# IDEA-CCNL/Fengshenbang-LM

Measured on NVIDIA H100. Metric: tokens_per_sec, higher is better.
Workload: dtype bf16

## Files before the change

### fengshen-lm_b200/csrc/gemm.cu

```cuda
#include "host_common.h"
#include "ptx.cuh"

namespace fsb {

constexpr int GEMM_BM = 128;
constexpr int GEMM_BK = 64;
constexpr int GEMM_THREADS = 384;

struct GemmParams {
  void* D;
  void* aux;
  const void* bias;
  int64_t ldd, ldaux, stride_d, stride_aux;
  int M, N, K, batch;
  int d_f32;
  int bias_f32;
  int epilogue;
  int accumulate;
  int tiles_m, tiles_n;
  int group_m;
  int ksplits;
};

template <int BN>
struct GemmSmem {
  static constexpr int STAGES = BN == 256 ? 4 : 6;
  static constexpr int A_BYTES = GEMM_BM * GEMM_BK * 2;
  static constexpr int B_BYTES = BN * GEMM_BK * 2;
  static constexpr int STAGE_BYTES = A_BYTES + B_BYTES;
  static constexpr int EPI_BUF_BYTES = 64 * 128;
  static constexpr int EPI_OFFSET = STAGES * STAGE_BYTES;
  static constexpr int BAR_OFFSET = EPI_OFFSET + 2  * 2  * EPI_BUF_BYTES;
  static constexpr int TOTAL = BAR_OFFSET + 2 * STAGES * 8 + 1024 ;
  static_assert(TOTAL <= kSmemOptIn, "exceeds the 227 KB of shared memory a block can opt into on sm_90");
};

__device__ __forceinline__ float gelu_tanh_f(float x) {
  const float k1 = 0.044715f, c = -2.f * 0.7978845608028654f * 1.4426950408889634f;
  const float t = ex2_approx(c * x * fmaf(k1, x * x, 1.f));
  return __fdividef(x, 1.f + t);
}
__device__ __forceinline__ float gelu_erf_f(float x) {
  const float z = fabsf(x) * 0.7071067811865476f;
  const float t = __fdividef(1.f, fmaf(0.3275911f, z, 1.f));
  float pl = fmaf(t, 1.061405429f, -1.453152027f);
  pl = fmaf(t, pl, 1.421413741f);
  pl = fmaf(t, pl, -0.284496736f);
  pl = fmaf(t, pl, 0.254829592f);
  const float erfc_z = pl * t * ex2_approx(-1.4426950408889634f * z * z);
  const float hx = 0.5f * x;
  return x >= 0.f ? fmaf(-hx, erfc_z, x) : hx * erfc_z;
}

__device__ __forceinline__ void tile_coords(int t, int tiles_m, int tiles_n, int group_m, int& b, int& m_idx, int& n_idx) {
  const int per = tiles_m * tiles_n;
  b = t / per;
  int r = t - b * per;
  const int group_span = group_m * tiles_n;
  const int g = r / group_span;
  const int first_m = g * group_m;
  const int gsize = min(tiles_m - first_m, group_m);
  const int in_g = r - g * group_span;
  m_idx = first_m + in_g % gsize;
  n_idx = in_g / gsize;
}

__device__ __forceinline__ void k_range(const GemmParams& p, int b, int num_kb, int& kb_lo, int& kb_hi, int& ab) {
  if (p.ksplits > 1) {
    kb_lo = int(int64_t(b) * num_kb / p.ksplits);
    kb_hi = int(int64_t(b + 1) * num_kb / p.ksplits);
    ab = 0;
  } else {
    kb_lo = 0; kb_hi = num_kb; ab = b;
  }
}

template <int kLayout, int BN>
__global__ void __launch_bounds__(GEMM_THREADS, 1)
gemm_bf16_kernel(const __grid_constant__ CUtensorMap tmA, const __grid_constant__ CUtensorMap tmB,
                 const __grid_constant__ CUtensorMap tmD, const __grid_constant__ CUtensorMap tmAux, const GemmParams p) {
  constexpr bool A_MN = (kLayout == FSB_GEMM_TN);
  constexpr bool B_MN = (kLayout != FSB_GEMM_NT);
  using S = GemmSmem<BN>;

  extern __shared__ uint8_t smem_raw[];
  uint8_t* smem = align_smem_1024(smem_raw);
  TmaRing<S::STAGES> ring(reinterpret_cast<uint64_t*>(smem + S::BAR_OFFSET));

  const int warp = threadIdx.x >> 5;
  const int lane = threadIdx.x & 31;
  const int num_tiles = p.tiles_m * p.tiles_n * p.batch;
  const int num_kb = (p.K + GEMM_BK - 1) / GEMM_BK;

  if (threadIdx.x == 0) {
    tma_prefetch_desc(&tmA);
    tma_prefetch_desc(&tmB);
    ring.init();
    fence_barrier_init();
  }
  if (threadIdx.x == 128) {
    tma_prefetch_desc(&tmD);
    if (p.aux != nullptr) tma_prefetch_desc(&tmAux);
  }
  __syncthreads();

  if (warp < 4) {
    reg_dec<40>();
    if (threadIdx.x == 0) {
      for (int t = blockIdx.x; t < num_tiles; t += gridDim.x) {
        int b, m_idx, n_idx, kb_lo, kb_hi, ab;
        tile_coords(t, p.tiles_m, p.tiles_n, p.group_m, b, m_idx, n_idx);
        k_range(p, b, num_kb, kb_lo, kb_hi, ab);
        const int m0 = m_idx * GEMM_BM, n0 = n_idx * BN;
        for (int kb = kb_lo; kb < kb_hi; ++kb) {
          ring.acquire();
          uint8_t* sa = smem + ring.stage * S::STAGE_BYTES;
          uint8_t* sb = sa + S::A_BYTES;
          uint64_t* bar = ring.expect(S::STAGE_BYTES);
          const int k0 = kb * GEMM_BK;
          if constexpr (!A_MN) {
            tma_load_3d(sa, &tmA, bar, k0, m0, ab);
          } else {
#pragma unroll
            for (int c = 0; c < GEMM_BM / 64; ++c)
              tma_load_3d(sa + c * (GEMM_BK * 128), &tmA, bar, m0 + c * 64, k0, ab);
          }
          if constexpr (!B_MN) {
            tma_load_3d(sb, &tmB, bar, k0, n0, ab);
          } else {
#pragma unroll
            for (int c = 0; c < BN / 64; ++c)
              tma_load_3d(sb + c * (GEMM_BK * 128), &tmB, bar, n0 + c * 64, k0, ab);
          }
          ring.advance();
        }
      }
    }
  } else {
    reg_inc<232>();
    const int wg = (threadIdx.x >> 7) - 1;
    const int wl = warp & 3;
    const bool leader = (threadIdx.x & 127) == 0;
    const uint64_t dsc_a = A_MN ? make_smem_desc_sw128(smem_u32(smem) + wg * (GEMM_BK * 128), GEMM_BK * 128, 1024)
                                : make_smem_desc_sw128(smem_u32(smem) + wg * (64 * 128), 0, 1024);
    const uint64_t dsc_b = B_MN ? make_smem_desc_sw128(smem_u32(smem) + S::A_BYTES, GEMM_BK * 128, 1024)
                                : make_smem_desc_sw128(smem_u32(smem) + S::A_BYTES, 0, 1024);
    uint8_t* const epi_buf = smem + S::EPI_OFFSET + wg * (2 * S::EPI_BUF_BYTES);
    uint32_t n_stored = 0;
    float acc[BN / 2];
    for (int t = blockIdx.x; t < num_tiles; t += gridDim.x) {
      int b, m_idx, n_idx, kb_lo, kb_hi, ab;
      tile_coords(t, p.tiles_m, p.tiles_n, p.group_m, b, m_idx, n_idx);
      k_range(p, b, num_kb, kb_lo, kb_hi, ab);
      int prev = 0;
      for (int kb = kb_lo; kb < kb_hi; ++kb) {
        ring.wait();
        const uint64_t so = uint64_t(ring.stage) * (S::STAGE_BYTES >> 4);
        wgmma_fence();
#pragma unroll
        for (int k = 0; k < GEMM_BK / 16; ++k) {
          const uint64_t da = dsc_a + so + ((A_MN ? k * 2048 : k * 32) >> 4), db = dsc_b + so + ((B_MN ? k * 2048 : k * 32) >> 4);
          const uint32_t accum = (kb != kb_lo || k != 0) ? 1u : 0u;
          if constexpr (BN == 256) wgmma_ss_n256<A_MN, B_MN>(acc, da, db, accum);
          else wgmma_ss_n128<A_MN, B_MN>(acc, da, db, accum);
        }
        wgmma_commit();
        wgmma_wait<1>();
        if (kb > kb_lo) ring.release(prev, lane);
        prev = ring.stage;
        ring.advance();
      }
      wgmma_wait<0>();
      wgmma_fence_acc(acc);
      ring.release(prev, lane);

      const int r = wl * 16 + (lane >> 2);
      const int m0 = m_idx * GEMM_BM + wg * 64, n0 = n_idx * BN;
      const int64_t d_off = int64_t(b) * p.stride_d;
      auto stage_out = [&](const CUtensorMap* tm, int c0, auto&& fill) {
        uint8_t* buf = epi_buf + (n_stored & 1) * S::EPI_BUF_BYTES;
        if (leader) tma_store_wait_read<1>();
        bar_sync(1 + wg, 128);
        fill(buf);
        fence_proxy_async();
        bar_sync(1 + wg, 128);
        if (leader) {
          tma_store_3d(tm, buf, c0, m0, b);
          tma_store_commit();
        }
        ++n_stored;
      };
#pragma unroll
      for (int j = 0; j < BN / 8; ++j) {
        const int col = n0 + 8 * j + 2 * (lane & 3);
        float bv0 = 0.f, bv1 = 0.f;
        if (p.bias != nullptr) {
          if (p.bias_f32) {
            if (col < p.N) bv0 = __ldg(reinterpret_cast<const float*>(p.bias) + col);
            if (col + 1 < p.N) bv1 = __ldg(reinterpret_cast<const float*>(p.bias) + col + 1);
          } else {
            if (col < p.N) bv0 = __bfloat162float(__ldg(reinterpret_cast<const __nv_bfloat16*>(p.bias) + col));
            if (col + 1 < p.N) bv1 = __bfloat162float(__ldg(reinterpret_cast<const __nv_bfloat16*>(p.bias) + col + 1));
          }
        }
        acc[4 * j] += bv0; acc[4 * j + 1] += bv1; acc[4 * j + 2] += bv0; acc[4 * j + 3] += bv1;
      }
#pragma unroll
      for (int g = 0; g < BN / 64; ++g) {
        if (p.aux != nullptr) {
          stage_out(&tmAux, n0 + 64 * g, [&](uint8_t* buf) {
#pragma unroll
            for (int jj = 0; jj < 8; ++jj)
#pragma unroll
              for (int h = 0; h < 2; ++h) {
                const int j = 8 * g + jj;
                *reinterpret_cast<uint32_t*>(buf + swz128(r + 8 * h, 16 * jj + 4 * (lane & 3))) =
                    pack_bf16x2(acc[4 * j + 2 * h], acc[4 * j + 2 * h + 1]);
              }
          });
        }
#pragma unroll
        for (int i = 32 * g; i < 32 * g + 32; ++i) {
          if (p.epilogue == FSB_EPI_GELU_TANH) acc[i] = gelu_tanh_f(acc[i]);
          else if (p.epilogue == FSB_EPI_GELU_ERF) acc[i] = gelu_erf_f(acc[i]);
        }
        if (p.accumulate) {
#pragma unroll
          for (int jj = 0; jj < 8; ++jj) {
            const int j = 8 * g + jj;
            const int col = n0 + 8 * j + 2 * (lane & 3);
#pragma unroll
            for (int h = 0; h < 2; ++h) {
              const int row = m0 + r + 8 * h;
              if (row >= p.M || col >= p.N) continue;
              const bool two = col + 1 < p.N;
              const int64_t o = d_off + int64_t(row) * p.ldd + col;
              if (p.d_f32) {
                const float* dp = reinterpret_cast<const float*>(p.D) + o;
                if (two) { const float2 q = *reinterpret_cast<const float2*>(dp); acc[4 * j + 2 * h] += q.x; acc[4 * j + 2 * h + 1] += q.y; }
                else acc[4 * j + 2 * h] += *dp;
              } else {
                const __nv_bfloat16* dp = reinterpret_cast<const __nv_bfloat16*>(p.D) + o;
                if (two) { const uint32_t q = *reinterpret_cast<const uint32_t*>(dp); acc[4 * j + 2 * h] += bf16lo(q); acc[4 * j + 2 * h + 1] += bf16hi(q); }
                else acc[4 * j + 2 * h] += __bfloat162float(*dp);
              }
            }
          }
        }
        if (p.d_f32) {
#pragma unroll
          for (int q = 0; q < 2; ++q)
            stage_out(&tmD, n0 + 64 * g + 32 * q, [&](uint8_t* buf) {
#pragma unroll
              for (int jj = 0; jj < 4; ++jj)
#pragma unroll
                for (int h = 0; h < 2; ++h) {
                  const int j = 8 * g + 4 * q + jj;
                  *reinterpret_cast<float2*>(buf + swz128(r + 8 * h, 32 * jj + 8 * (lane & 3))) =
                      make_float2(acc[4 * j + 2 * h], acc[4 * j + 2 * h + 1]);
                }
            });
        } else {
          stage_out(&tmD, n0 + 64 * g, [&](uint8_t* buf) {
#pragma unroll
            for (int jj = 0; jj < 8; ++jj)
#pragma unroll
              for (int h = 0; h < 2; ++h) {
                const int j = 8 * g + jj;
                *reinterpret_cast<uint32_t*>(buf + swz128(r + 8 * h, 16 * jj + 4 * (lane & 3))) =
                    pack_bf16x2(acc[4 * j + 2 * h], acc[4 * j + 2 * h + 1]);
              }
          });
        }
      }
    }
    if (leader) tma_store_wait<0>();
  }
}

static int g_reserved_sms = 0;
static inline int gemm_sms() {
  const int n = num_sms() - g_reserved_sms;
  return n < 1 ? 1 : n;
}

template <int kLayout, int BN>
static int launch_gemm(const CUtensorMap& tmA, const CUtensorMap& tmB, const CUtensorMap& tmD, const CUtensorMap& tmAux,
                       const GemmParams& p, cudaStream_t stream) {
  using S = GemmSmem<BN>;
  if (int rc = ensure_smem<gemm_bf16_kernel<kLayout, BN>>(S::TOTAL, "gemm")) return rc;
  const int num_tiles = p.tiles_m * p.tiles_n * p.batch;
  const int grid = num_tiles < gemm_sms() ? num_tiles : gemm_sms();
  gemm_bf16_kernel<kLayout, BN><<<grid, GEMM_THREADS, S::TOTAL, stream>>>(tmA, tmB, tmD, tmAux, p);
  FSB_CUDA_LAUNCH_CHECK();
  return FSB_OK;
}

struct GemmPlan {
  int bn, splits;
};
static GemmPlan gemm_plan(int layout, int64_t M, int64_t N, int64_t K, int64_t batch, bool plain, int sms) {
  const int64_t tiles256 = ((M + GEMM_BM - 1) / GEMM_BM) * ((N + 255) / 256) * batch;
  const int bn = (N > 128 && tiles256 * 10 >= int64_t(sms) * 7) ? 256 : 128;
  if (!(layout == FSB_GEMM_TN && batch == 1 && plain && N % 4 == 0 && (M * N) % 8 == 0 && K >= 4096)) return {bn, 1};
  const bool wide = N >= 256;
  const int64_t tiles = ((M + GEMM_BM - 1) / GEMM_BM) * (wide ? (N + 255) / 256 : (N + 127) / 128);
  int splits = int(sms / tiles);
  if (splits > 16) splits = 16;
  while (splits > 1 && (K % (int64_t(splits) * GEMM_BK) != 0 || K / splits < 1024)) --splits;
  if (splits >= 2 && tiles * 2 <= sms) return {wide ? 256 : bn, splits};
  return {bn, 1};
}

__global__ void splitk_reduce_kernel(const float* __restrict__ ws, int splits, int64_t M, int64_t N, void* D, int64_t ldd,
                                     int d_f32, int accumulate) {
  const int64_t n4 = N / 4;
  for (int64_t i = blockIdx.x * int64_t(blockDim.x) + threadIdx.x; i < M * n4; i += int64_t(gridDim.x) * blockDim.x) {
    const int64_t m = i / n4, n = (i - m * n4) * 4;
    float4 acc = *reinterpret_cast<const float4*>(ws + m * N + n);
    for (int s = 1; s < splits; ++s) {
      const float4 v = *reinterpret_cast<const float4*>(ws + (int64_t(s) * M + m) * N + n);
      acc.x += v.x; acc.y += v.y; acc.z += v.z; acc.w += v.w;
    }
    if (d_f32) {
      float4* dp = reinterpret_cast<float4*>(reinterpret_cast<float*>(D) + m * ldd + n);
      if (accumulate) { const float4 o = *dp; acc.x += o.x; acc.y += o.y; acc.z += o.z; acc.w += o.w; }
      *dp = acc;
    } else {
      uint2* dp = reinterpret_cast<uint2*>(reinterpret_cast<__nv_bfloat16*>(D) + m * ldd + n);
      if (accumulate) {
        const uint2 o = *dp;
        acc.x += bf16lo(o.x); acc.y += bf16hi(o.x); acc.z += bf16lo(o.y); acc.w += bf16hi(o.y);
      }
      *dp = make_uint2(pack_bf16x2(acc.x, acc.y), pack_bf16x2(acc.z, acc.w));
    }
  }
}

static int gemm_impl(int layout, int64_t M, int64_t N, int64_t K, const void* A, int64_t lda, const void* B,
                     int64_t ldb, void* D, int64_t ldd, int d_dtype, const void* bias, int bias_dtype,
                     int epilogue, int accumulate, void* aux, int64_t ldaux, int64_t batch, int64_t stride_a,
                     int64_t stride_b, int64_t stride_d, int64_t stride_aux, cudaStream_t stream, int bn = 0,
                     int ksplits = 1);

}

using namespace fsb;

extern "C" int fsb_set_reserved_sms(int n) {
  FSB_REQUIRE(n >= 0 && n <= 64, "set_reserved_sms: %d out of range [0, 64]", n);
  fsb::g_reserved_sms = n;
  return FSB_OK;
}

extern "C" size_t fsb_gemm_workspace_bytes(int layout, int64_t M, int64_t N, int64_t K) {
  if (M <= 0 || N <= 0 || K <= 0) return 0;
  const int splits = gemm_plan(layout, M, N, K, 1, true, gemm_sms()).splits;
  return splits > 1 ? size_t(splits) * size_t(M) * size_t(N) * sizeof(float) : 0;
}

extern "C" int fsb_gemm_bf16(int layout, int64_t M, int64_t N, int64_t K, const void* A, int64_t lda, const void* B,
                             int64_t ldb, void* D, int64_t ldd, int d_dtype, const void* bias, int bias_dtype,
                             int epilogue, int accumulate, void* aux, int64_t ldaux, int64_t batch, int64_t stride_a,
                             int64_t stride_b, int64_t stride_d, int64_t stride_aux, void* workspace,
                             size_t workspace_bytes, fsb_stream_t stream_) {
  cudaStream_t stream = static_cast<cudaStream_t>(stream_);
  FSB_REQUIRE(M > 0 && N > 0 && K > 0 && batch > 0, "gemm: non-positive dims M=%ld N=%ld K=%ld batch=%ld", (long)M,
              (long)N, (long)K, (long)batch);
  const GemmPlan plan = gemm_plan(layout, M, N, K, batch, bias == nullptr && aux == nullptr && epilogue == FSB_EPI_NONE,
                                  gemm_sms());
  if (plan.splits > 1 && (d_dtype == FSB_BF16 || d_dtype == FSB_F32)) {
    const int splits = plan.splits;
    const size_t need = size_t(splits) * size_t(M) * size_t(N) * sizeof(float);
    FSB_REQUIRE(workspace != nullptr && workspace_bytes >= need && aligned16(workspace),
                "gemm: this TN call splits K %d ways and needs a %zu-byte workspace (fsb_gemm_workspace_bytes); got %zu",
                splits, need, workspace_bytes);
    FSB_REQUIRE(ldd % 4 == 0, "gemm: ldd=%ld not vector-aligned", (long)ldd);
    float* ws = static_cast<float*>(workspace);
    int rc = gemm_impl(layout, M, N, K, A, lda, B, ldb, ws, N, FSB_F32, nullptr, FSB_BF16, FSB_EPI_NONE, 0, nullptr, 0,
                       splits, 0, 0, M * N, 0, stream, plan.bn, splits);
    if (rc) return rc;
    const int64_t work = M * (N / 4);
    const int blocks = int(work / 256 + 1 < 2 * num_sms() ? work / 256 + 1 : 2 * num_sms());
    splitk_reduce_kernel<<<blocks, 256, 0, stream>>>(ws, splits, M, N, D, ldd, d_dtype == FSB_F32, accumulate);
    FSB_CUDA_LAUNCH_CHECK();
    return FSB_OK;
  }
  return gemm_impl(layout, M, N, K, A, lda, B, ldb, D, ldd, d_dtype, bias, bias_dtype, epilogue, accumulate, aux, ldaux, batch,
                   stride_a, stride_b, stride_d, stride_aux, stream, plan.bn, 1);
}

static int fsb::gemm_impl(int layout, int64_t M, int64_t N, int64_t K, const void* A, int64_t lda, const void* B,
                          int64_t ldb, void* D, int64_t ldd, int d_dtype, const void* bias, int bias_dtype,
                          int epilogue, int accumulate, void* aux, int64_t ldaux, int64_t batch, int64_t stride_a,
                          int64_t stride_b, int64_t stride_d, int64_t stride_aux, cudaStream_t stream, int bn,
                          int ksplits) {
  FSB_REQUIRE(layout >= 0 && layout <= 2, "gemm: bad layout %d", layout);
  FSB_REQUIRE(M > 0 && N > 0 && K > 0 && batch > 0, "gemm: non-positive dims M=%ld N=%ld K=%ld batch=%ld", (long)M,
              (long)N, (long)K, (long)batch);
  FSB_REQUIRE(M < (1 << 30) && N < (1 << 30) && K < (1 << 30), "gemm: dims too large");
  FSB_REQUIRE(A && B && D, "gemm: null operand");
  FSB_REQUIRE(aligned16(A) && aligned16(B) && aligned16(D), "gemm: operands must be 16-byte aligned");
  FSB_REQUIRE(lda % 8 == 0 && ldb % 8 == 0, "gemm: lda/ldb must be multiples of 8 (lda=%ld ldb=%ld)", (long)lda,
              (long)ldb);
  FSB_REQUIRE(d_dtype == FSB_BF16 || d_dtype == FSB_F32, "gemm: bad d_dtype");
  FSB_REQUIRE(ldd % (d_dtype == FSB_F32 ? 4 : 8) == 0, "gemm: ldd=%ld not vector-aligned", (long)ldd);
  FSB_REQUIRE(epilogue >= 0 && epilogue <= 2, "gemm: bad epilogue %d", epilogue);
  FSB_REQUIRE(aux == nullptr || (aligned16(aux) && ldaux % 8 == 0), "gemm: aux misaligned");
  FSB_REQUIRE(batch == 1 || (stride_a % 8 == 0 && stride_b % 8 == 0 && stride_d % 8 == 0),
              "gemm: batch strides must be multiples of 8");
  FSB_REQUIRE(aux == nullptr || batch == 1 || stride_aux % 8 == 0, "gemm: aux batch stride must be a multiple of 8");
  FSB_REQUIRE(ksplits == 1 || (ksplits > 1 && ksplits <= (K + GEMM_BK - 1) / GEMM_BK && ksplits == batch),
              "gemm: bad K-split count %d", ksplits);

  CUtensorMap tmA, tmB, tmD, tmAux;
  const bool a_mn = (layout == FSB_GEMM_TN), b_mn = (layout != FSB_GEMM_NT);
  const int BN = bn ? bn : gemm_plan(layout, M, N, K, batch, false, gemm_sms()).bn;
  const int64_t ab = ksplits > 1 ? 1 : batch;
  {
    uint64_t dims[3] = {uint64_t(a_mn ? M : K), uint64_t(a_mn ? K : M), uint64_t(ab)};
    uint64_t strides[2] = {uint64_t(lda) * 2, uint64_t(ab > 1 ? stride_a : (a_mn ? K : M) * lda) * 2};
    uint32_t box[3] = {64, uint32_t(a_mn ? GEMM_BK : GEMM_BM), 1};
    int rc = make_tmap_bf16(&tmA, A, 3, dims, strides, box);
    if (rc) return rc;
  }
  {
    uint64_t dims[3] = {uint64_t(b_mn ? N : K), uint64_t(b_mn ? K : N), uint64_t(ab)};
    uint64_t strides[2] = {uint64_t(ldb) * 2, uint64_t(ab > 1 ? stride_b : (b_mn ? K : N) * ldb) * 2};
    uint32_t box[3] = {64, uint32_t(b_mn ? GEMM_BK : BN), 1};
    int rc = make_tmap_bf16(&tmB, B, 3, dims, strides, box);
    if (rc) return rc;
  }
  {
    const int64_t es = d_dtype == FSB_F32 ? 4 : 2;
    uint64_t dims[3] = {uint64_t(N), uint64_t(M), uint64_t(batch)};
    uint64_t strides[2] = {uint64_t(ldd * es), uint64_t((batch > 1 ? stride_d : M * ldd) * es)};
    uint32_t box[3] = {uint32_t(128 / es), 64, 1};
    int rc = d_dtype == FSB_F32 ? make_tmap_f32(&tmD, D, 3, dims, strides, box) : make_tmap_bf16(&tmD, D, 3, dims, strides, box);
    if (rc) return rc;
    if (aux != nullptr) {
      uint64_t astrides[2] = {uint64_t(ldaux * 2), uint64_t((batch > 1 ? stride_aux : M * ldaux) * 2)};
      uint32_t abox[3] = {64, 64, 1};
      rc = make_tmap_bf16(&tmAux, aux, 3, dims, astrides, abox);
      if (rc) return rc;
    } else {
      tmAux = tmD;
    }
  }
  GemmParams p;
  p.D = D; p.aux = aux; p.bias = bias;
  p.ldd = ldd; p.ldaux = ldaux; p.stride_d = stride_d; p.stride_aux = stride_aux;
  p.M = int(M); p.N = int(N); p.K = int(K); p.batch = int(batch);
  p.d_f32 = (d_dtype == FSB_F32); p.bias_f32 = (bias_dtype == FSB_F32);
  p.epilogue = epilogue; p.accumulate = accumulate;
  p.ksplits = ksplits;
  p.tiles_m = int((M + GEMM_BM - 1) / GEMM_BM);
  p.tiles_n = int((N + BN - 1) / BN);
  {
    const int64_t a_panel = int64_t(GEMM_BM) * (K / ksplits) * 2;
    const int64_t base = BN == 256 ? 16 : 12;
    int64_t gm = (int64_t(32) << 20) / a_panel;
    gm = gm < base ? base : (gm > 64 ? 64 : gm);
    p.group_m = int(gm);
  }

#define FSB_GEMM_DISPATCH(L) \
  case L:                    \
    return BN == 256 ? launch_gemm<L, 256>(tmA, tmB, tmD, tmAux, p, stream) : launch_gemm<L, 128>(tmA, tmB, tmD, tmAux, p, stream);
  switch (layout) {
    FSB_GEMM_DISPATCH(FSB_GEMM_NT)
    FSB_GEMM_DISPATCH(FSB_GEMM_NN)
    FSB_GEMM_DISPATCH(FSB_GEMM_TN)
  }
#undef FSB_GEMM_DISPATCH
  return FSB_ERR_INVALID;
}
```

### fengshen-lm_b200/csrc/ptx.cuh

```cuda
#pragma once
#include <cuda.h>
#include <cuda_bf16.h>
#include <cuda_runtime.h>
#include <stdint.h>

namespace fsb {

__device__ __forceinline__ uint32_t smem_u32(const void* p) {
  return static_cast<uint32_t>(__cvta_generic_to_shared(p));
}

__device__ __forceinline__ void mbar_init(uint64_t* bar, uint32_t count) {
  asm volatile("mbarrier.init.shared::cta.b64 [%0], %1;" ::"r"(smem_u32(bar)), "r"(count) : "memory");
}
__device__ __forceinline__ void fence_barrier_init() {
  asm volatile("fence.mbarrier_init.release.cluster;" ::: "memory");
}
__device__ __forceinline__ void fence_proxy_async() {
  asm volatile("fence.proxy.async.shared::cta;" ::: "memory");
}
__device__ __forceinline__ void mbar_expect_tx(uint64_t* bar, uint32_t bytes) {
  asm volatile("mbarrier.arrive.expect_tx.shared::cta.b64 _, [%0], %1;" ::"r"(smem_u32(bar)), "r"(bytes)
               : "memory");
}
__device__ __forceinline__ void mbar_arrive(uint64_t* bar) {
  asm volatile("mbarrier.arrive.shared::cta.b64 _, [%0];" ::"r"(smem_u32(bar)) : "memory");
}
__device__ __forceinline__ bool mbar_try_wait(uint64_t* bar, uint32_t parity) {
  uint32_t ok;
  asm volatile(
      "{\n\t"
      ".reg .pred p;\n\t"
      "mbarrier.try_wait.parity.shared::cta.b64 p, [%1], %2;\n\t"
      "selp.b32 %0, 1, 0, p;\n\t"
      "}"
      : "=r"(ok)
      : "r"(smem_u32(bar)), "r"(parity)
      : "memory");
  return ok != 0;
}
__device__ __forceinline__ bool mbar_test(uint64_t* bar, uint32_t parity) {
  uint32_t ok;
  asm volatile(
      "{\n\t"
      ".reg .pred p;\n\t"
      "mbarrier.test_wait.parity.shared::cta.b64 p, [%1], %2;\n\t"
      "selp.b32 %0, 1, 0, p;\n\t"
      "}"
      : "=r"(ok)
      : "r"(smem_u32(bar)), "r"(parity)
      : "memory");
  return ok != 0;
}
__device__ __forceinline__ void mbar_wait(uint64_t* bar, uint32_t parity) {
  while (!mbar_try_wait(bar, parity)) {
  }
}

constexpr int kSmemOptIn = 232448;

__device__ __forceinline__ uint8_t* align_smem_1024(uint8_t* smem_raw) {
  return reinterpret_cast<uint8_t*>((reinterpret_cast<uintptr_t>(smem_raw) + 1023) & ~uintptr_t(1023));
}

template <int STAGES, int NFULL = 1>
struct TmaRing {
  uint64_t* const bar;
  uint64_t* const empty_bar;
  int stage = 0;
  uint32_t phase = 0;

  __device__ __forceinline__ explicit TmaRing(uint64_t* bars) : bar(bars), empty_bar(bars + NFULL * STAGES) {}
  __device__ __forceinline__ uint64_t* full(int f) const { return bar + f * STAGES + stage; }
  __device__ __forceinline__ uint64_t* empty(int s) const { return empty_bar + s; }

  __device__ __forceinline__ void init() const {
    for (int s = 0; s < STAGES; ++s) {
      for (int f = 0; f < NFULL; ++f) mbar_init(bar + f * STAGES + s, 1);
      mbar_init(empty(s), 8);
    }
  }
  __device__ __forceinline__ void acquire() const { mbar_wait(empty(stage), phase ^ 1); }
  __device__ __forceinline__ uint64_t* expect(uint32_t bytes, int f = 0) const {
    mbar_expect_tx(full(f), bytes);
    return full(f);
  }
  __device__ __forceinline__ void wait(int f = 0) const { mbar_wait(full(f), phase); }
  __device__ __forceinline__ void release(int s, int lane) const {
    if (lane == 0) mbar_arrive(empty(s));
  }
  __device__ __forceinline__ void release(int lane) const { release(stage, lane); }
  __device__ __forceinline__ void advance() {
    if (++stage == STAGES) { stage = 0; phase ^= 1; }
  }
  __device__ __forceinline__ TmaRing at(int j) const {
    TmaRing r(bar);
    r.stage = j % STAGES;
    r.phase = (j / STAGES) & 1;
    return r;
  }
};

__device__ __forceinline__ void tma_prefetch_desc(const CUtensorMap* m) {
  asm volatile("prefetch.tensormap [%0];" ::"l"(reinterpret_cast<uint64_t>(m)) : "memory");
}
__device__ __forceinline__ void tma_load_2d(void* smem_dst, const CUtensorMap* m, uint64_t* bar, int c0, int c1) {
  asm volatile(
      "cp.async.bulk.tensor.2d.shared::cluster.global.mbarrier::complete_tx::bytes [%0], [%1, {%3, %4}], [%2];"
      ::"r"(smem_u32(smem_dst)), "l"(reinterpret_cast<uint64_t>(m)), "r"(smem_u32(bar)), "r"(c0), "r"(c1)
      : "memory");
}
__device__ __forceinline__ void tma_load_3d(void* smem_dst, const CUtensorMap* m, uint64_t* bar, int c0, int c1,
                                            int c2) {
  asm volatile(
      "cp.async.bulk.tensor.3d.shared::cluster.global.mbarrier::complete_tx::bytes [%0], [%1, {%3, %4, %5}], [%2];"
      ::"r"(smem_u32(smem_dst)), "l"(reinterpret_cast<uint64_t>(m)), "r"(smem_u32(bar)), "r"(c0), "r"(c1), "r"(c2)
      : "memory");
}
__device__ __forceinline__ void tma_store_2d(const CUtensorMap* m, const void* smem_src, int c0, int c1) {
  asm volatile("cp.async.bulk.tensor.2d.global.shared::cta.bulk_group [%0, {%2, %3}], [%1];" ::"l"(
                   reinterpret_cast<uint64_t>(m)),
               "r"(smem_u32(smem_src)), "r"(c0), "r"(c1)
               : "memory");
}
__device__ __forceinline__ void tma_store_3d(const CUtensorMap* m, const void* smem_src, int c0, int c1, int c2) {
  asm volatile("cp.async.bulk.tensor.3d.global.shared::cta.bulk_group [%0, {%2, %3, %4}], [%1];" ::"l"(
                   reinterpret_cast<uint64_t>(m)),
               "r"(smem_u32(smem_src)), "r"(c0), "r"(c1), "r"(c2)
               : "memory");
}
__device__ __forceinline__ void tma_store_commit() { asm volatile("cp.async.bulk.commit_group;" ::: "memory"); }
template <int N>
__device__ __forceinline__ void tma_store_wait_read() {
  asm volatile("cp.async.bulk.wait_group.read %0;" ::"n"(N) : "memory");
}
template <int N>
__device__ __forceinline__ void tma_store_wait() {
  asm volatile("cp.async.bulk.wait_group %0;" ::"n"(N) : "memory");
}

__device__ __forceinline__ void wgmma_fence() { asm volatile("wgmma.fence.sync.aligned;" ::: "memory"); }
__device__ __forceinline__ void wgmma_commit() { asm volatile("wgmma.commit_group.sync.aligned;" ::: "memory"); }
template <int N>
__device__ __forceinline__ void wgmma_wait() { asm volatile("wgmma.wait_group.sync.aligned %0;" ::"n"(N) : "memory"); }
template <int R>
__device__ __forceinline__ void wgmma_fence_acc(float (&d)[R]) {
#pragma unroll
  for (int i = 0; i < R; ++i) asm volatile("" : "+f"(d[i])::"memory");
}
template <int N> __device__ __forceinline__ void reg_inc() { asm volatile("setmaxnreg.inc.sync.aligned.u32 %0;" ::"n"(N)); }
template <int N> __device__ __forceinline__ void reg_dec() { asm volatile("setmaxnreg.dec.sync.aligned.u32 %0;" ::"n"(N)); }
__device__ __forceinline__ void bar_sync(int id, int n) { asm volatile("bar.sync %0, %1;" ::"r"(id), "r"(n) : "memory"); }
__device__ __forceinline__ float ex2_approx(float x) {
  float y;
  asm("ex2.approx.ftz.f32 %0, %1;" : "=f"(y) : "f"(x));
  return y;
}

__device__ __forceinline__ uint64_t make_smem_desc_sw128(uint32_t saddr, uint32_t lbo, uint32_t sbo) {
  uint64_t d = 0;
  d |= static_cast<uint64_t>((saddr & 0x3FFFF) >> 4);
  d |= static_cast<uint64_t>((lbo >> 4) & 0x3FFF) << 16;
  d |= static_cast<uint64_t>((sbo >> 4) & 0x3FFF) << 32;
  d |= static_cast<uint64_t>(1) << 62;
  return d;
}
__device__ __forceinline__ uint32_t swz128(int row, int byte) {
  return uint32_t(row * 128 + ((((byte >> 4) ^ row) & 7) << 4) + (byte & 15));
}

template <int kTB>
__device__ __forceinline__ void wgmma_rs_n8(float (&d)[4], const uint32_t (&a)[4], uint64_t db, uint32_t accumulate) {
  asm volatile(
      "{\n.reg .pred p;\nsetp.ne.b32 p, %9, 0;\n"
      "wgmma.mma_async.sync.aligned.m64n8k16.f32.bf16.bf16 {%0, %1, %2, %3}, {%4, %5, %6, %7}, %8, p, 1, 1, %10;\n}"
      : "+f"(d[0]), "+f"(d[1]), "+f"(d[2]), "+f"(d[3])
      : "r"(a[0]), "r"(a[1]), "r"(a[2]), "r"(a[3]), "l"(db), "r"(accumulate), "n"(kTB));
}
template <int kTB>
__device__ __forceinline__ void wgmma_rs_n16(float (&d)[8], const uint32_t (&a)[4], uint64_t db, uint32_t accumulate) {
  asm volatile(
      "{\n.reg .pred p;\nsetp.ne.b32 p, %13, 0;\n"
      "wgmma.mma_async.sync.aligned.m64n16k16.f32.bf16.bf16 {%0, %1, %2, %3, %4, %5, %6, %7}, {%8, %9, %10, %11}, %12, p, 1, 1, %14;\n}"
      : "+f"(d[0]), "+f"(d[1]), "+f"(d[2]), "+f"(d[3]), "+f"(d[4]), "+f"(d[5]), "+f"(d[6]), "+f"(d[7])
      : "r"(a[0]), "r"(a[1]), "r"(a[2]), "r"(a[3]), "l"(db), "r"(accumulate), "n"(kTB));
}
template <int kTB>
__device__ __forceinline__ void wgmma_rs_n32(float (&d)[16], const uint32_t (&a)[4], uint64_t db, uint32_t accumulate) {
  asm volatile(
      "{\n.reg .pred p;\nsetp.ne.b32 p, %21, 0;\n"
      "wgmma.mma_async.sync.aligned.m64n32k16.f32.bf16.bf16 {%0, %1, %2, %3, %4, %5, %6, %7, %8, %9, %10, %11, %12, %13, %14, %15}, {%16, %17, %18, %19}, %20, p, 1, 1, %22;\n}"
      : "+f"(d[0]), "+f"(d[1]), "+f"(d[2]), "+f"(d[3]), "+f"(d[4]), "+f"(d[5]), "+f"(d[6]), "+f"(d[7]), "+f"(d[8]), "+f"(d[9]), "+f"(d[10]), "+f"(d[11]), "+f"(d[12]), "+f"(d[13]), "+f"(d[14]), "+f"(d[15])
      : "r"(a[0]), "r"(a[1]), "r"(a[2]), "r"(a[3]), "l"(db), "r"(accumulate), "n"(kTB));
}
template <int kTA, int kTB>
__device__ __forceinline__ void wgmma_ss_n64(float (&d)[32], uint64_t da, uint64_t db, uint32_t accumulate) {
  asm volatile(
      "{\n.reg .pred p;\nsetp.ne.b32 p, %34, 0;\n"
      "wgmma.mma_async.sync.aligned.m64n64k16.f32.bf16.bf16 {%0, %1, %2, %3, %4, %5, %6, %7, %8, %9, %10, %11, %12, %13, %14, %15, %16, %17, %18, %19, %20, %21, %22, %23, %24, %25, %26, %27, %28, %29, %30, %31}, %32, %33, p, 1, 1, %35, %36;\n}"
      : "+f"(d[0]), "+f"(d[1]), "+f"(d[2]), "+f"(d[3]), "+f"(d[4]), "+f"(d[5]), "+f"(d[6]), "+f"(d[7]), "+f"(d[8]), "+f"(d[9]), "+f"(d[10]), "+f"(d[11]), "+f"(d[12]), "+f"(d[13]), "+f"(d[14]), "+f"(d[15]), "+f"(d[16]), "+f"(d[17]), "+f"(d[18]), "+f"(d[19]), "+f"(d[20]), "+f"(d[21]), "+f"(d[22]), "+f"(d[23]), "+f"(d[24]), "+f"(d[25]), "+f"(d[26]), "+f"(d[27]), "+f"(d[28]), "+f"(d[29]), "+f"(d[30]), "+f"(d[31])
      : "l"(da), "l"(db), "r"(accumulate), "n"(kTA), "n"(kTB));
}
template <int kTB>
__device__ __forceinline__ void wgmma_rs_n64(float (&d)[32], const uint32_t (&a)[4], uint64_t db, uint32_t accumulate) {
  asm volatile(
      "{\n.reg .pred p;\nsetp.ne.b32 p, %37, 0;\n"
      "wgmma.mma_async.sync.aligned.m64n64k16.f32.bf16.bf16 {%0, %1, %2, %3, %4, %5, %6, %7, %8, %9, %10, %11, %12, %13, %14, %15, %16, %17, %18, %19, %20, %21, %22, %23, %24, %25, %26, %27, %28, %29, %30, %31}, {%32, %33, %34, %35}, %36, p, 1, 1, %38;\n}"
      : "+f"(d[0]), "+f"(d[1]), "+f"(d[2]), "+f"(d[3]), "+f"(d[4]), "+f"(d[5]), "+f"(d[6]), "+f"(d[7]), "+f"(d[8]), "+f"(d[9]), "+f"(d[10]), "+f"(d[11]), "+f"(d[12]), "+f"(d[13]), "+f"(d[14]), "+f"(d[15]), "+f"(d[16]), "+f"(d[17]), "+f"(d[18]), "+f"(d[19]), "+f"(d[20]), "+f"(d[21]), "+f"(d[22]), "+f"(d[23]), "+f"(d[24]), "+f"(d[25]), "+f"(d[26]), "+f"(d[27]), "+f"(d[28]), "+f"(d[29]), "+f"(d[30]), "+f"(d[31])
      : "r"(a[0]), "r"(a[1]), "r"(a[2]), "r"(a[3]), "l"(db), "r"(accumulate), "n"(kTB));
}
template <int kTA, int kTB>
__device__ __forceinline__ void wgmma_ss_n128(float (&d)[64], uint64_t da, uint64_t db, uint32_t accumulate) {
  asm volatile(
      "{\n.reg .pred p;\nsetp.ne.b32 p, %66, 0;\n"
      "wgmma.mma_async.sync.aligned.m64n128k16.f32.bf16.bf16 {%0, %1, %2, %3, %4, %5, %6, %7, %8, %9, %10, %11, %12, %13, %14, %15, %16, %17, %18, %19, %20, %21, %22, %23, %24, %25, %26, %27, %28, %29, %30, %31, %32, %33, %34, %35, %36, %37, %38, %39, %40, %41, %42, %43, %44, %45, %46, %47, %48, %49, %50, %51, %52, %53, %54, %55, %56, %57, %58, %59, %60, %61, %62, %63}, %64, %65, p, 1, 1, %67, %68;\n}"
      : "+f"(d[0]), "+f"(d[1]), "+f"(d[2]), "+f"(d[3]), "+f"(d[4]), "+f"(d[5]), "+f"(d[6]), "+f"(d[7]), "+f"(d[8]), "+f"(d[9]), "+f"(d[10]), "+f"(d[11]), "+f"(d[12]), "+f"(d[13]), "+f"(d[14]), "+f"(d[15]), "+f"(d[16]), "+f"(d[17]), "+f"(d[18]), "+f"(d[19]), "+f"(d[20]), "+f"(d[21]), "+f"(d[22]), "+f"(d[23]), "+f"(d[24]), "+f"(d[25]), "+f"(d[26]), "+f"(d[27]), "+f"(d[28]), "+f"(d[29]), "+f"(d[30]), "+f"(d[31]), "+f"(d[32]), "+f"(d[33]), "+f"(d[34]), "+f"(d[35]), "+f"(d[36]), "+f"(d[37]), "+f"(d[38]), "+f"(d[39]), "+f"(d[40]), "+f"(d[41]), "+f"(d[42]), "+f"(d[43]), "+f"(d[44]), "+f"(d[45]), "+f"(d[46]), "+f"(d[47]), "+f"(d[48]), "+f"(d[49]), "+f"(d[50]), "+f"(d[51]), "+f"(d[52]), "+f"(d[53]), "+f"(d[54]), "+f"(d[55]), "+f"(d[56]), "+f"(d[57]), "+f"(d[58]), "+f"(d[59]), "+f"(d[60]), "+f"(d[61]), "+f"(d[62]), "+f"(d[63])
      : "l"(da), "l"(db), "r"(accumulate), "n"(kTA), "n"(kTB));
}
template <int kTB>
__device__ __forceinline__ void wgmma_rs_n128(float (&d)[64], const uint32_t (&a)[4], uint64_t db, uint32_t accumulate) {
  asm volatile(
      "{\n.reg .pred p;\nsetp.ne.b32 p, %69, 0;\n"
      "wgmma.mma_async.sync.aligned.m64n128k16.f32.bf16.bf16 {%0, %1, %2, %3, %4, %5, %6, %7, %8, %9, %10, %11, %12, %13, %14, %15, %16, %17, %18, %19, %20, %21, %22, %23, %24, %25, %26, %27, %28, %29, %30, %31, %32, %33, %34, %35, %36, %37, %38, %39, %40, %41, %42, %43, %44, %45, %46, %47, %48, %49, %50, %51, %52, %53, %54, %55, %56, %57, %58, %59, %60, %61, %62, %63}, {%64, %65, %66, %67}, %68, p, 1, 1, %70;\n}"
      : "+f"(d[0]), "+f"(d[1]), "+f"(d[2]), "+f"(d[3]), "+f"(d[4]), "+f"(d[5]), "+f"(d[6]), "+f"(d[7]), "+f"(d[8]), "+f"(d[9]), "+f"(d[10]), "+f"(d[11]), "+f"(d[12]), "+f"(d[13]), "+f"(d[14]), "+f"(d[15]), "+f"(d[16]), "+f"(d[17]), "+f"(d[18]), "+f"(d[19]), "+f"(d[20]), "+f"(d[21]), "+f"(d[22]), "+f"(d[23]), "+f"(d[24]), "+f"(d[25]), "+f"(d[26]), "+f"(d[27]), "+f"(d[28]), "+f"(d[29]), "+f"(d[30]), "+f"(d[31]), "+f"(d[32]), "+f"(d[33]), "+f"(d[34]), "+f"(d[35]), "+f"(d[36]), "+f"(d[37]), "+f"(d[38]), "+f"(d[39]), "+f"(d[40]), "+f"(d[41]), "+f"(d[42]), "+f"(d[43]), "+f"(d[44]), "+f"(d[45]), "+f"(d[46]), "+f"(d[47]), "+f"(d[48]), "+f"(d[49]), "+f"(d[50]), "+f"(d[51]), "+f"(d[52]), "+f"(d[53]), "+f"(d[54]), "+f"(d[55]), "+f"(d[56]), "+f"(d[57]), "+f"(d[58]), "+f"(d[59]), "+f"(d[60]), "+f"(d[61]), "+f"(d[62]), "+f"(d[63])
      : "r"(a[0]), "r"(a[1]), "r"(a[2]), "r"(a[3]), "l"(db), "r"(accumulate), "n"(kTB));
}
template <int kTA, int kTB>
__device__ __forceinline__ void wgmma_ss_n256(float (&d)[128], uint64_t da, uint64_t db, uint32_t accumulate) {
  asm volatile(
      "{\n.reg .pred p;\nsetp.ne.b32 p, %130, 0;\n"
      "wgmma.mma_async.sync.aligned.m64n256k16.f32.bf16.bf16 {%0, %1, %2, %3, %4, %5, %6, %7, %8, %9, %10, %11, %12, %13, %14, %15, %16, %17, %18, %19, %20, %21, %22, %23, %24, %25, %26, %27, %28, %29, %30, %31, %32, %33, %34, %35, %36, %37, %38, %39, %40, %41, %42, %43, %44, %45, %46, %47, %48, %49, %50, %51, %52, %53, %54, %55, %56, %57, %58, %59, %60, %61, %62, %63, %64, %65, %66, %67, %68, %69, %70, %71, %72, %73, %74, %75, %76, %77, %78, %79, %80, %81, %82, %83, %84, %85, %86, %87, %88, %89, %90, %91, %92, %93, %94, %95, %96, %97, %98, %99, %100, %101, %102, %103, %104, %105, %106, %107, %108, %109, %110, %111, %112, %113, %114, %115, %116, %117, %118, %119, %120, %121, %122, %123, %124, %125, %126, %127}, %128, %129, p, 1, 1, %131, %132;\n}"
      : "+f"(d[0]), "+f"(d[1]), "+f"(d[2]), "+f"(d[3]), "+f"(d[4]), "+f"(d[5]), "+f"(d[6]), "+f"(d[7]), "+f"(d[8]), "+f"(d[9]), "+f"(d[10]), "+f"(d[11]), "+f"(d[12]), "+f"(d[13]), "+f"(d[14]), "+f"(d[15]), "+f"(d[16]), "+f"(d[17]), "+f"(d[18]), "+f"(d[19]), "+f"(d[20]), "+f"(d[21]), "+f"(d[22]), "+f"(d[23]), "+f"(d[24]), "+f"(d[25]), "+f"(d[26]), "+f"(d[27]), "+f"(d[28]), "+f"(d[29]), "+f"(d[30]), "+f"(d[31]), "+f"(d[32]), "+f"(d[33]), "+f"(d[34]), "+f"(d[35]), "+f"(d[36]), "+f"(d[37]), "+f"(d[38]), "+f"(d[39]), "+f"(d[40]), "+f"(d[41]), "+f"(d[42]), "+f"(d[43]), "+f"(d[44]), "+f"(d[45]), "+f"(d[46]), "+f"(d[47]), "+f"(d[48]), "+f"(d[49]), "+f"(d[50]), "+f"(d[51]), "+f"(d[52]), "+f"(d[53]), "+f"(d[54]), "+f"(d[55]), "+f"(d[56]), "+f"(d[57]), "+f"(d[58]), "+f"(d[59]), "+f"(d[60]), "+f"(d[61]), "+f"(d[62]), "+f"(d[63]), "+f"(d[64]), "+f"(d[65]), "+f"(d[66]), "+f"(d[67]), "+f"(d[68]), "+f"(d[69]), "+f"(d[70]), "+f"(d[71]), "+f"(d[72]), "+f"(d[73]), "+f"(d[74]), "+f"(d[75]), "+f"(d[76]), "+f"(d[77]), "+f"(d[78]), "+f"(d[79]), "+f"(d[80]), "+f"(d[81]), "+f"(d[82]), "+f"(d[83]), "+f"(d[84]), "+f"(d[85]), "+f"(d[86]), "+f"(d[87]), "+f"(d[88]), "+f"(d[89]), "+f"(d[90]), "+f"(d[91]), "+f"(d[92]), "+f"(d[93]), "+f"(d[94]), "+f"(d[95]), "+f"(d[96]), "+f"(d[97]), "+f"(d[98]), "+f"(d[99]), "+f"(d[100]), "+f"(d[101]), "+f"(d[102]), "+f"(d[103]), "+f"(d[104]), "+f"(d[105]), "+f"(d[106]), "+f"(d[107]), "+f"(d[108]), "+f"(d[109]), "+f"(d[110]), "+f"(d[111]), "+f"(d[112]), "+f"(d[113]), "+f"(d[114]), "+f"(d[115]), "+f"(d[116]), "+f"(d[117]), "+f"(d[118]), "+f"(d[119]), "+f"(d[120]), "+f"(d[121]), "+f"(d[122]), "+f"(d[123]), "+f"(d[124]), "+f"(d[125]), "+f"(d[126]), "+f"(d[127])
      : "l"(da), "l"(db), "r"(accumulate), "n"(kTA), "n"(kTB));
}
template <int kTB>
__device__ __forceinline__ void wgmma_rs_n256(float (&d)[128], const uint32_t (&a)[4], uint64_t db, uint32_t accumulate) {
  asm volatile(
      "{\n.reg .pred p;\nsetp.ne.b32 p, %133, 0;\n"
      "wgmma.mma_async.sync.aligned.m64n256k16.f32.bf16.bf16 {%0, %1, %2, %3, %4, %5, %6, %7, %8, %9, %10, %11, %12, %13, %14, %15, %16, %17, %18, %19, %20, %21, %22, %23, %24, %25, %26, %27, %28, %29, %30, %31, %32, %33, %34, %35, %36, %37, %38, %39, %40, %41, %42, %43, %44, %45, %46, %47, %48, %49, %50, %51, %52, %53, %54, %55, %56, %57, %58, %59, %60, %61, %62, %63, %64, %65, %66, %67, %68, %69, %70, %71, %72, %73, %74, %75, %76, %77, %78, %79, %80, %81, %82, %83, %84, %85, %86, %87, %88, %89, %90, %91, %92, %93, %94, %95, %96, %97, %98, %99, %100, %101, %102, %103, %104, %105, %106, %107, %108, %109, %110, %111, %112, %113, %114, %115, %116, %117, %118, %119, %120, %121, %122, %123, %124, %125, %126, %127}, {%128, %129, %130, %131}, %132, p, 1, 1, %134;\n}"
      : "+f"(d[0]), "+f"(d[1]), "+f"(d[2]), "+f"(d[3]), "+f"(d[4]), "+f"(d[5]), "+f"(d[6]), "+f"(d[7]), "+f"(d[8]), "+f"(d[9]), "+f"(d[10]), "+f"(d[11]), "+f"(d[12]), "+f"(d[13]), "+f"(d[14]), "+f"(d[15]), "+f"(d[16]), "+f"(d[17]), "+f"(d[18]), "+f"(d[19]), "+f"(d[20]), "+f"(d[21]), "+f"(d[22]), "+f"(d[23]), "+f"(d[24]), "+f"(d[25]), "+f"(d[26]), "+f"(d[27]), "+f"(d[28]), "+f"(d[29]), "+f"(d[30]), "+f"(d[31]), "+f"(d[32]), "+f"(d[33]), "+f"(d[34]), "+f"(d[35]), "+f"(d[36]), "+f"(d[37]), "+f"(d[38]), "+f"(d[39]), "+f"(d[40]), "+f"(d[41]), "+f"(d[42]), "+f"(d[43]), "+f"(d[44]), "+f"(d[45]), "+f"(d[46]), "+f"(d[47]), "+f"(d[48]), "+f"(d[49]), "+f"(d[50]), "+f"(d[51]), "+f"(d[52]), "+f"(d[53]), "+f"(d[54]), "+f"(d[55]), "+f"(d[56]), "+f"(d[57]), "+f"(d[58]), "+f"(d[59]), "+f"(d[60]), "+f"(d[61]), "+f"(d[62]), "+f"(d[63]), "+f"(d[64]), "+f"(d[65]), "+f"(d[66]), "+f"(d[67]), "+f"(d[68]), "+f"(d[69]), "+f"(d[70]), "+f"(d[71]), "+f"(d[72]), "+f"(d[73]), "+f"(d[74]), "+f"(d[75]), "+f"(d[76]), "+f"(d[77]), "+f"(d[78]), "+f"(d[79]), "+f"(d[80]), "+f"(d[81]), "+f"(d[82]), "+f"(d[83]), "+f"(d[84]), "+f"(d[85]), "+f"(d[86]), "+f"(d[87]), "+f"(d[88]), "+f"(d[89]), "+f"(d[90]), "+f"(d[91]), "+f"(d[92]), "+f"(d[93]), "+f"(d[94]), "+f"(d[95]), "+f"(d[96]), "+f"(d[97]), "+f"(d[98]), "+f"(d[99]), "+f"(d[100]), "+f"(d[101]), "+f"(d[102]), "+f"(d[103]), "+f"(d[104]), "+f"(d[105]), "+f"(d[106]), "+f"(d[107]), "+f"(d[108]), "+f"(d[109]), "+f"(d[110]), "+f"(d[111]), "+f"(d[112]), "+f"(d[113]), "+f"(d[114]), "+f"(d[115]), "+f"(d[116]), "+f"(d[117]), "+f"(d[118]), "+f"(d[119]), "+f"(d[120]), "+f"(d[121]), "+f"(d[122]), "+f"(d[123]), "+f"(d[124]), "+f"(d[125]), "+f"(d[126]), "+f"(d[127])
      : "r"(a[0]), "r"(a[1]), "r"(a[2]), "r"(a[3]), "l"(db), "r"(accumulate), "n"(kTB));
}
template <int N, int kTB>
__device__ __forceinline__ void wgmma_rs_dim(float (&d)[N / 2], const uint32_t (&a)[4], uint64_t db, uint32_t accumulate) {
  static_assert(N == 8 || N == 16 || N == 32 || N == 64 || N == 128 || N == 256, "no m64nNk16 wgmma for this N");
  if constexpr (N == 8) wgmma_rs_n8<kTB>(d, a, db, accumulate);
  else if constexpr (N == 16) wgmma_rs_n16<kTB>(d, a, db, accumulate);
  else if constexpr (N == 32) wgmma_rs_n32<kTB>(d, a, db, accumulate);
  else if constexpr (N == 64) wgmma_rs_n64<kTB>(d, a, db, accumulate);
  else if constexpr (N == 128) wgmma_rs_n128<kTB>(d, a, db, accumulate);
  else wgmma_rs_n256<kTB>(d, a, db, accumulate);
}

__device__ __forceinline__ uint32_t pack_bf16x2(float lo, float hi) {
  __nv_bfloat162 v = __floats2bfloat162_rn(lo, hi);
  return *reinterpret_cast<uint32_t*>(&v);
}
__device__ __forceinline__ float bf16lo(uint32_t u) { return __uint_as_float(u << 16); }
__device__ __forceinline__ float bf16hi(uint32_t u) { return __uint_as_float(u & 0xFFFF0000u); }

__device__ __forceinline__ void unpack8(const uint4& q, float (&f)[8]) {
  f[0] = bf16lo(q.x); f[1] = bf16hi(q.x); f[2] = bf16lo(q.y); f[3] = bf16hi(q.y);
  f[4] = bf16lo(q.z); f[5] = bf16hi(q.z); f[6] = bf16lo(q.w); f[7] = bf16hi(q.w);
}
__device__ __forceinline__ uint4 pack8(const float (&f)[8]) {
  uint4 q;
  q.x = pack_bf16x2(f[0], f[1]); q.y = pack_bf16x2(f[2], f[3]);
  q.z = pack_bf16x2(f[4], f[5]); q.w = pack_bf16x2(f[6], f[7]);
  return q;
}
__device__ __forceinline__ float round_bf16(float x) { return __bfloat162float(__float2bfloat16(x)); }
__device__ __forceinline__ uint32_t lds_u16(uint32_t addr) {
  uint16_t v;
  asm volatile("ld.shared.u16 %0, [%1];" : "=h"(v) : "r"(addr));
  return v;
}
__device__ __forceinline__ uint32_t lds_u32(uint32_t addr) {
  uint32_t v;
  asm volatile("ld.shared.u32 %0, [%1];" : "=r"(v) : "r"(addr));
  return v;
}

}
```

Before: 449,500.

## Add ping-pong GEMM schedule for short-K tiles and a BN=192 tile option

Adds a ping-pong consumer mode for K up to 1024 when there are at least twice as many 128x128 tiles as SMs. Each consumer warpgroup computes a whole 128x128 tile in turn, and named barriers hand the mainloop to the other warpgroup so one group's epilogue overlaps the other's MMAs. The planner also gains a BN=192 tile (new m64n192 wgmma wrapper) picked when it reduces the wave-quantized work per SM, and the epilogue moves into a shared helper. The cost is more accumulator registers per warpgroup in ping-pong mode, plus extra barrier handoffs and ring-indexing complexity.

```diff
diff --git a/fengshen-lm_b200/csrc/gemm.cu b/fengshen-lm_b200/csrc/gemm.cu
--- a/fengshen-lm_b200/csrc/gemm.cu
+++ b/fengshen-lm_b200/csrc/gemm.cu
@@ -6,6 +6,7 @@
 constexpr int GEMM_BM = 128;
 constexpr int GEMM_BK = 64;
 constexpr int GEMM_THREADS = 384;
+constexpr int GEMM_PINGPONG_MAX_K = 1024;
 
 struct GemmParams {
   void* D;
@@ -24,7 +25,7 @@
 
 template <int BN>
 struct GemmSmem {
-  static constexpr int STAGES = BN == 256 ? 4 : 6;
+  static constexpr int STAGES = BN == 128 ? 6 : 4;
   static constexpr int A_BYTES = GEMM_BM * GEMM_BK * 2;
   static constexpr int B_BYTES = BN * GEMM_BK * 2;
   static constexpr int STAGE_BYTES = A_BYTES + B_BYTES;
@@ -75,17 +76,125 @@
   }
 }
 
-template <int kLayout, int BN>
+template <int NC>
+__device__ __forceinline__ void epilogue_rows64(float (&acc)[NC / 2], const GemmParams& p, const CUtensorMap* tmD,
+                                                const CUtensorMap* tmAux, int b, int m0, int n0, uint8_t* epi_buf,
+                                                uint32_t& n_stored, int wg, bool leader) {
+  constexpr int BUF_BYTES = GemmSmem<NC>::EPI_BUF_BYTES;
+  const int lane = threadIdx.x & 31;
+  const int r = ((threadIdx.x >> 5) & 3) * 16 + (lane >> 2);
+  const int64_t d_off = int64_t(b) * p.stride_d;
+  auto stage_out = [&](const CUtensorMap* tm, int c0, auto&& fill) {
+    uint8_t* buf = epi_buf + (n_stored & 1) * BUF_BYTES;
+    if (leader) tma_store_wait_read<1>();
+    bar_sync(1 + wg, 128);
+    fill(buf);
+    fence_proxy_async();
+    bar_sync(1 + wg, 128);
+    if (leader) {
+      tma_store_3d(tm, buf, c0, m0, b);
+      tma_store_commit();
+    }
+    ++n_stored;
+  };
+#pragma unroll
+  for (int j = 0; j < NC / 8; ++j) {
+    const int col = n0 + 8 * j + 2 * (lane & 3);
+    float bv0 = 0.f, bv1 = 0.f;
+    if (p.bias != nullptr) {
+      if (p.bias_f32) {
+        if (col < p.N) bv0 = __ldg(reinterpret_cast<const float*>(p.bias) + col);
+        if (col + 1 < p.N) bv1 = __ldg(reinterpret_cast<const float*>(p.bias) + col + 1);
+      } else {
+        if (col < p.N) bv0 = __bfloat162float(__ldg(reinterpret_cast<const __nv_bfloat16*>(p.bias) + col));
+        if (col + 1 < p.N) bv1 = __bfloat162float(__ldg(reinterpret_cast<const __nv_bfloat16*>(p.bias) + col + 1));
+      }
+    }
+    acc[4 * j] += bv0; acc[4 * j + 1] += bv1; acc[4 * j + 2] += bv0; acc[4 * j + 3] += bv1;
+  }
+#pragma unroll
+  for (int g = 0; g < NC / 64; ++g) {
+    if (p.aux != nullptr) {
+      stage_out(tmAux, n0 + 64 * g, [&](uint8_t* buf) {
+#pragma unroll
+        for (int jj = 0; jj < 8; ++jj)
+#pragma unroll
+          for (int h = 0; h < 2; ++h) {
+            const int j = 8 * g + jj;
+            *reinterpret_cast<uint32_t*>(buf + swz128(r + 8 * h, 16 * jj + 4 * (lane & 3))) =
+                pack_bf16x2(acc[4 * j + 2 * h], acc[4 * j + 2 * h + 1]);
+          }
+      });
+    }
+#pragma unroll
+    for (int i = 32 * g; i < 32 * g + 32; ++i) {
+      if (p.epilogue == FSB_EPI_GELU_TANH) acc[i] = gelu_tanh_f(acc[i]);
+      else if (p.epilogue == FSB_EPI_GELU_ERF) acc[i] = gelu_erf_f(acc[i]);
+    }
+    if (p.accumulate) {
+#pragma unroll
+      for (int jj = 0; jj < 8; ++jj) {
+        const int j = 8 * g + jj;
+        const int col = n0 + 8 * j + 2 * (lane & 3);
+#pragma unroll
+        for (int h = 0; h < 2; ++h) {
+          const int row = m0 + r + 8 * h;
+          if (row >= p.M || col >= p.N) continue;
+          const bool two = col + 1 < p.N;
+          const int64_t o = d_off + int64_t(row) * p.ldd + col;
+          if (p.d_f32) {
+            const float* dp = reinterpret_cast<const float*>(p.D) + o;
+            if (two) { const float2 q = *reinterpret_cast<const float2*>(dp); acc[4 * j + 2 * h] += q.x; acc[4 * j + 2 * h + 1] += q.y; }
+            else acc[4 * j + 2 * h] += *dp;
+          } else {
+            const __nv_bfloat16* dp = reinterpret_cast<const __nv_bfloat16*>(p.D) + o;
+            if (two) { const uint32_t q = *reinterpret_cast<const uint32_t*>(dp); acc[4 * j + 2 * h] += bf16lo(q); acc[4 * j + 2 * h + 1] += bf16hi(q); }
+            else acc[4 * j + 2 * h] += __bfloat162float(*dp);
+          }
+        }
+      }
+    }
+    if (p.d_f32) {
+#pragma unroll
+      for (int q = 0; q < 2; ++q)
+        stage_out(tmD, n0 + 64 * g + 32 * q, [&](uint8_t* buf) {
+#pragma unroll
+          for (int jj = 0; jj < 4; ++jj)
+#pragma unroll
+            for (int h = 0; h < 2; ++h) {
+              const int j = 8 * g + 4 * q + jj;
+              *reinterpret_cast<float2*>(buf + swz128(r + 8 * h, 32 * jj + 8 * (lane & 3))) =
+                  make_float2(acc[4 * j + 2 * h], acc[4 * j + 2 * h + 1]);
+            }
+        });
+    } else {
+      stage_out(tmD, n0 + 64 * g, [&](uint8_t* buf) {
+#pragma unroll
+        for (int jj = 0; jj < 8; ++jj)
+#pragma unroll
+          for (int h = 0; h < 2; ++h) {
+            const int j = 8 * g + jj;
+            *reinterpret_cast<uint32_t*>(buf + swz128(r + 8 * h, 16 * jj + 4 * (lane & 3))) =
+                pack_bf16x2(acc[4 * j + 2 * h], acc[4 * j + 2 * h + 1]);
+          }
+      });
+    }
+  }
+}
+
+template <int kLayout, int BN, bool kPingPong>
 __global__ void __launch_bounds__(GEMM_THREADS, 1)
 gemm_bf16_kernel(const __grid_constant__ CUtensorMap tmA, const __grid_constant__ CUtensorMap tmB,
                  const __grid_constant__ CUtensorMap tmD, const __grid_constant__ CUtensorMap tmAux, const GemmParams p) {
   constexpr bool A_MN = (kLayout == FSB_GEMM_TN);
   constexpr bool B_MN = (kLayout != FSB_GEMM_NT);
+  static_assert(!kPingPong || BN == 128, "ping-pong tiles are 128 x 128");
+  constexpr int MI = kPingPong ? 2 : 1;
   using S = GemmSmem<BN>;
 
   extern __shared__ uint8_t smem_raw[];
   uint8_t* smem = align_smem_1024(smem_raw);
-  TmaRing<S::STAGES> ring(reinterpret_cast<uint64_t*>(smem + S::BAR_OFFSET));
+  TmaRing<S::STAGES, 1, kPingPong ? 4 : 8> ring(reinterpret_cast<uint64_t*>(smem + S::BAR_OFFSET));
 
   const int warp = threadIdx.x >> 5;
   const int lane = threadIdx.x & 31;
@@ -139,140 +248,56 @@
   } else {
     reg_inc<232>();
     const int wg = (threadIdx.x >> 7) - 1;
-    const int wl = warp & 3;
     const bool leader = (threadIdx.x & 127) == 0;
-    const uint64_t dsc_a = A_MN ? make_smem_desc_sw128(smem_u32(smem) + wg * (GEMM_BK * 128), GEMM_BK * 128, 1024)
-                                : make_smem_desc_sw128(smem_u32(smem) + wg * (64 * 128), 0, 1024);
+    uint64_t dsc_a[MI];
+#pragma unroll
+    for (int mi = 0; mi < MI; ++mi) {
+      const int h = kPingPong ? mi : wg;
+      dsc_a[mi] = A_MN ? make_smem_desc_sw128(smem_u32(smem) + h * (GEMM_BK * 128), GEMM_BK * 128, 1024)
+                       : make_smem_desc_sw128(smem_u32(smem) + h * (64 * 128), 0, 1024);
+    }
     const uint64_t dsc_b = B_MN ? make_smem_desc_sw128(smem_u32(smem) + S::A_BYTES, GEMM_BK * 128, 1024)
                                 : make_smem_desc_sw128(smem_u32(smem) + S::A_BYTES, 0, 1024);
     uint8_t* const epi_buf = smem + S::EPI_OFFSET + wg * (2 * S::EPI_BUF_BYTES);
     uint32_t n_stored = 0;
-    float acc[BN / 2];
-    for (int t = blockIdx.x; t < num_tiles; t += gridDim.x) {
+    int kb_seen = 0;
+    float acc[MI][BN / 2];
+    for (int t = blockIdx.x, i = 0; t < num_tiles; t += gridDim.x, ++i) {
       int b, m_idx, n_idx, kb_lo, kb_hi, ab;
       tile_coords(t, p.tiles_m, p.tiles_n, p.group_m, b, m_idx, n_idx);
       k_range(p, b, num_kb, kb_lo, kb_hi, ab);
+      auto rg = ring.at(kb_seen);
+      kb_seen += kb_hi - kb_lo;
+      if (kPingPong && (i & 1) != wg) continue;
+      if (kPingPong && i > 0) bar_sync(3 + wg, 256);
       int prev = 0;
       for (int kb = kb_lo; kb < kb_hi; ++kb) {
-        ring.wait();
-        const uint64_t so = uint64_t(ring.stage) * (S::STAGE_BYTES >> 4);
+        rg.wait();
+        const uint64_t so = uint64_t(rg.stage) * (S::STAGE_BYTES >> 4);
         wgmma_fence();
 #pragma unroll
         for (int k = 0; k < GEMM_BK / 16; ++k) {
-          const uint64_t da = dsc_a + so + ((A_MN ? k * 2048 : k * 32) >> 4), db = dsc_b + so + ((B_MN ? k * 2048 : k * 32) >> 4);
+          const uint64_t db = dsc_b + so + ((B_MN ? k * 2048 : k * 32) >> 4);
           const uint32_t accum = (kb != kb_lo || k != 0) ? 1u : 0u;
-          if constexpr (BN == 256) wgmma_ss_n256<A_MN, B_MN>(acc, da, db, accum);
-          else wgmma_ss_n128<A_MN, B_MN>(acc, da, db, accum);
+#pragma unroll
+          for (int mi = 0; mi < MI; ++mi)
+            wgmma_ss_dim<BN, A_MN, B_MN>(acc[mi], dsc_a[mi] + so + ((A_MN ? k * 2048 : k * 32) >> 4), db, accum);
         }
         wgmma_commit();
         wgmma_wait<1>();
-        if (kb > kb_lo) ring.release(prev, lane);
-        prev = ring.stage;
-        ring.advance();
+        if (kb > kb_lo) rg.release(prev, lane);
+        prev = rg.stage;
+        rg.advance();
       }
+      if (kPingPong && t + int(gridDim.x) < num_tiles) bar_arrive(3 + (wg ^ 1), 256);
       wgmma_wait<0>();
-      wgmma_fence_acc(acc);
-      ring.release(prev, lane);
-
-      const int r = wl * 16 + (lane >> 2);
-      const int m0 = m_idx * GEMM_BM + wg * 64, n0 = n_idx * BN;
-      const int64_t d_off = int64_t(b) * p.stride_d;
-      auto stage_out = [&](const CUtensorMap* tm, int c0, auto&& fill) {
-        uint8_t* buf = epi_buf + (n_stored & 1) * S::EPI_BUF_BYTES;
-        if (leader) tma_store_wait_read<1>();
-        bar_sync(1 + wg, 128);
-        fill(buf);
-        fence_proxy_async();
-        bar_sync(1 + wg, 128);
-        if (leader) {
-          tma_store_3d(tm, buf, c0, m0, b);
-          tma_store_commit();
-        }
-        ++n_stored;
-      };
-#pragma unroll
-      for (int j = 0; j < BN / 8; ++j) {
-        const int col = n0 + 8 * j + 2 * (lane & 3);
-        float bv0 = 0.f, bv1 = 0.f;
-        if (p.bias != nullptr) {
-          if (p.bias_f32) {
-            if (col < p.N) bv0 = __ldg(reinterpret_cast<const float*>(p.bias) + col);
-            if (col + 1 < p.N) bv1 = __ldg(reinterpret_cast<const float*>(p.bias) + col + 1);
-          } else {
-            if (col < p.N) bv0 = __bfloat162float(__ldg(reinterpret_cast<const __nv_bfloat16*>(p.bias) + col));
-            if (col + 1 < p.N) bv1 = __bfloat162float(__ldg(reinterpret_cast<const __nv_bfloat16*>(p.bias) + col + 1));
-          }
-        }
-        acc[4 * j] += bv0; acc[4 * j + 1] += bv1; acc[4 * j + 2] += bv0; acc[4 * j + 3] += bv1;
-      }
-#pragma unroll
-      for (int g = 0; g < BN / 64; ++g) {
-        if (p.aux != nullptr) {
-          stage_out(&tmAux, n0 + 64 * g, [&](uint8_t* buf) {
-#pragma unroll
-            for (int jj = 0; jj < 8; ++jj)
-#pragma unroll
-              for (int h = 0; h < 2; ++h) {
-                const int j = 8 * g + jj;
-                *reinterpret_cast<uint32_t*>(buf + swz128(r + 8 * h, 16 * jj + 4 * (lane & 3))) =
-                    pack_bf16x2(acc[4 * j + 2 * h], acc[4 * j + 2 * h + 1]);
-              }
-          });
-        }
-#pragma unroll
-        for (int i = 32 * g; i < 32 * g + 32; ++i) {
-          if (p.epilogue == FSB_EPI_GELU_TANH) acc[i] = gelu_tanh_f(acc[i]);
-          else if (p.epilogue == FSB_EPI_GELU_ERF) acc[i] = gelu_erf_f(acc[i]);
-        }
-        if (p.accumulate) {
-#pragma unroll
-          for (int jj = 0; jj < 8; ++jj) {
-            const int j = 8 * g + jj;
-            const int col = n0 + 8 * j + 2 * (lane & 3);
-#pragma unroll
-            for (int h = 0; h < 2; ++h) {
-              const int row = m0 + r + 8 * h;
-              if (row >= p.M || col >= p.N) continue;
-              const bool two = col + 1 < p.N;
-              const int64_t o = d_off + int64_t(row) * p.ldd + col;
-              if (p.d_f32) {
-                const float* dp = reinterpret_cast<const float*>(p.D) + o;
-                if (two) { const float2 q = *reinterpret_cast<const float2*>(dp); acc[4 * j + 2 * h] += q.x; acc[4 * j + 2 * h + 1] += q.y; }
-                else acc[4 * j + 2 * h] += *dp;
-              } else {
-                const __nv_bfloat16* dp = reinterpret_cast<const __nv_bfloat16*>(p.D) + o;
-                if (two) { const uint32_t q = *reinterpret_cast<const uint32_t*>(dp); acc[4 * j + 2 * h] += bf16lo(q); acc[4 * j + 2 * h + 1] += bf16hi(q); }
-                else acc[4 * j + 2 * h] += __bfloat162float(*dp);
-              }
-            }
-          }
-        }
-        if (p.d_f32) {
-#pragma unroll
-          for (int q = 0; q < 2; ++q)
-            stage_out(&tmD, n0 + 64 * g + 32 * q, [&](uint8_t* buf) {
-#pragma unroll
-              for (int jj = 0; jj < 4; ++jj)
-#pragma unroll
-                for (int h = 0; h < 2; ++h) {
-                  const int j = 8 * g + 4 * q + jj;
-                  *reinterpret_cast<float2*>(buf + swz128(r + 8 * h, 32 * jj + 8 * (lane & 3))) =
-                      make_float2(acc[4 * j + 2 * h], acc[4 * j + 2 * h + 1]);
-                }
-            });
-        } else {
-          stage_out(&tmD, n0 + 64 * g, [&](uint8_t* buf) {
-#pragma unroll
-            for (int jj = 0; jj < 8; ++jj)
-#pragma unroll
-              for (int h = 0; h < 2; ++h) {
-                const int j = 8 * g + jj;
-                *reinterpret_cast<uint32_t*>(buf + swz128(r + 8 * h, 16 * jj + 4 * (lane & 3))) =
-                    pack_bf16x2(acc[4 * j + 2 * h], acc[4 * j + 2 * h + 1]);
-              }
-          });
-        }
-      }
+#pragma unroll
+      for (int mi = 0; mi < MI; ++mi) wgmma_fence_acc(acc[mi]);
+      rg.release(prev, lane);
+#pragma unroll
+      for (int mi = 0; mi < MI; ++mi)
+        epilogue_rows64<BN>(acc[mi], p, &tmD, &tmAux, b, m_idx * GEMM_BM + 64 * (kPingPong ? mi : wg), n_idx * BN, epi_buf,
+                            n_stored, wg, leader);
     }
     if (leader) tma_store_wait<0>();
   }
@@ -284,32 +309,41 @@
   return n < 1 ? 1 : n;
 }
 
-template <int kLayout, int BN>
+template <int kLayout, int BN, bool kPingPong>
 static int launch_gemm(const CUtensorMap& tmA, const CUtensorMap& tmB, const CUtensorMap& tmD, const CUtensorMap& tmAux,
                        const GemmParams& p, cudaStream_t stream) {
   using S = GemmSmem<BN>;
-  if (int rc = ensure_smem<gemm_bf16_kernel<kLayout, BN>>(S::TOTAL, "gemm")) return rc;
+  if (int rc = ensure_smem<gemm_bf16_kernel<kLayout, BN, kPingPong>>(S::TOTAL, "gemm")) return rc;
   const int num_tiles = p.tiles_m * p.tiles_n * p.batch;
   const int grid = num_tiles < gemm_sms() ? num_tiles : gemm_sms();
-  gemm_bf16_kernel<kLayout, BN><<<grid, GEMM_THREADS, S::TOTAL, stream>>>(tmA, tmB, tmD, tmAux, p);
+  gemm_bf16_kernel<kLayout, BN, kPingPong><<<grid, GEMM_THREADS, S::TOTAL, stream>>>(tmA, tmB, tmD, tmAux, p);
   FSB_CUDA_LAUNCH_CHECK();
   return FSB_OK;
 }
 
 struct GemmPlan {
   int bn, splits;
+  bool pingpong;
 };
 static GemmPlan gemm_plan(int layout, int64_t M, int64_t N, int64_t K, int64_t batch, bool plain, int sms) {
-  const int64_t tiles256 = ((M + GEMM_BM - 1) / GEMM_BM) * ((N + 255) / 256) * batch;
-  const int bn = (N > 128 && tiles256 * 10 >= int64_t(sms) * 7) ? 256 : 128;
-  if (!(layout == FSB_GEMM_TN && batch == 1 && plain && N % 4 == 0 && (M * N) % 8 == 0 && K >= 4096)) return {bn, 1};
+  const int64_t tiles_m = (M + GEMM_BM - 1) / GEMM_BM;
+  auto tiles = [&](int w) { return tiles_m * ((N + w - 1) / w) * batch; };
+  if (K <= GEMM_PINGPONG_MAX_K && tiles(128) >= 2 * int64_t(sms)) return {128, 1, true};
+  const int bn = (N > 128 && tiles(256) * 10 >= int64_t(sms) * 7) ? 256 : 128;
+  int bw = bn;
+  if (tiles(bn) > sms && tiles(bn) <= 2 * int64_t(sms)) {
+    auto work = [&](int w) { return (tiles(w) + sms - 1) / sms * w; };
+    for (int w : {128, 192, 256})
+      if (work(w) < work(bw)) bw = w;
+  }
+  if (!(layout == FSB_GEMM_TN && batch == 1 && plain && N % 4 == 0 && (M * N) % 8 == 0 && K >= 4096)) return {bw, 1, false};
   const bool wide = N >= 256;
-  const int64_t tiles = ((M + GEMM_BM - 1) / GEMM_BM) * (wide ? (N + 255) / 256 : (N + 127) / 128);
-  int splits = int(sms / tiles);
+  const int64_t split_tiles = tiles_m * (wide ? (N + 255) / 256 : (N + 127) / 128);
+  int splits = int(sms / split_tiles);
   if (splits > 16) splits = 16;
   while (splits > 1 && (K % (int64_t(splits) * GEMM_BK) != 0 || K / splits < 1024)) --splits;
-  if (splits >= 2 && tiles * 2 <= sms) return {wide ? 256 : bn, splits};
-  return {bn, 1};
+  if (splits >= 2 && split_tiles * 2 <= sms) return {wide ? 256 : bn, splits, false};
+  return {bw, 1, false};
 }
 
 __global__ void splitk_reduce_kernel(const float* __restrict__ ws, int splits, int64_t M, int64_t N, void* D, int64_t ldd,
@@ -340,8 +374,7 @@
 static int gemm_impl(int layout, int64_t M, int64_t N, int64_t K, const void* A, int64_t lda, const void* B,
                      int64_t ldb, void* D, int64_t ldd, int d_dtype, const void* bias, int bias_dtype,
                      int epilogue, int accumulate, void* aux, int64_t ldaux, int64_t batch, int64_t stride_a,
-                     int64_t stride_b, int64_t stride_d, int64_t stride_aux, cudaStream_t stream, int bn = 0,
-                     int ksplits = 1);
+                     int64_t stride_b, int64_t stride_d, int64_t stride_aux, cudaStream_t stream, GemmPlan plan);
 
 }
 
@@ -378,7 +411,7 @@
     FSB_REQUIRE(ldd % 4 == 0, "gemm: ldd=%ld not vector-aligned", (long)ldd);
     float* ws = static_cast<float*>(workspace);
     int rc = gemm_impl(layout, M, N, K, A, lda, B, ldb, ws, N, FSB_F32, nullptr, FSB_BF16, FSB_EPI_NONE, 0, nullptr, 0,
-                       splits, 0, 0, M * N, 0, stream, plan.bn, splits);
+                       splits, 0, 0, M * N, 0, stream, plan);
     if (rc) return rc;
     const int64_t work = M * (N / 4);
     const int blocks = int(work / 256 + 1 < 2 * num_sms() ? work / 256 + 1 : 2 * num_sms());
@@ -387,14 +420,14 @@
     return FSB_OK;
   }
   return gemm_impl(layout, M, N, K, A, lda, B, ldb, D, ldd, d_dtype, bias, bias_dtype, epilogue, accumulate, aux, ldaux, batch,
-                   stride_a, stride_b, stride_d, stride_aux, stream, plan.bn, 1);
+                   stride_a, stride_b, stride_d, stride_aux, stream, {plan.bn, 1, plan.pingpong});
 }
 
 static int fsb::gemm_impl(int layout, int64_t M, int64_t N, int64_t K, const void* A, int64_t lda, const void* B,
                           int64_t ldb, void* D, int64_t ldd, int d_dtype, const void* bias, int bias_dtype,
                           int epilogue, int accumulate, void* aux, int64_t ldaux, int64_t batch, int64_t stride_a,
-                          int64_t stride_b, int64_t stride_d, int64_t stride_aux, cudaStream_t stream, int bn,
-                          int ksplits) {
+                          int64_t stride_b, int64_t stride_d, int64_t stride_aux, cudaStream_t stream, GemmPlan plan) {
+  const int ksplits = plan.splits;
   FSB_REQUIRE(layout >= 0 && layout <= 2, "gemm: bad layout %d", layout);
   FSB_REQUIRE(M > 0 && N > 0 && K > 0 && batch > 0, "gemm: non-positive dims M=%ld N=%ld K=%ld batch=%ld", (long)M,
               (long)N, (long)K, (long)batch);
@@ -415,7 +448,7 @@
 
   CUtensorMap tmA, tmB, tmD, tmAux;
   const bool a_mn = (layout == FSB_GEMM_TN), b_mn = (layout != FSB_GEMM_NT);
-  const int BN = bn ? bn : gemm_plan(layout, M, N, K, batch, false, gemm_sms()).bn;
+  const int BN = plan.bn;
   const int64_t ab = ksplits > 1 ? 1 : batch;
   {
     uint64_t dims[3] = {uint64_t(a_mn ? M : K), uint64_t(a_mn ? K : M), uint64_t(ab)};
@@ -466,7 +499,10 @@
 
 #define FSB_GEMM_DISPATCH(L) \
   case L:                    \
-    return BN == 256 ? launch_gemm<L, 256>(tmA, tmB, tmD, tmAux, p, stream) : launch_gemm<L, 128>(tmA, tmB, tmD, tmAux, p, stream);
+    if (plan.pingpong) return launch_gemm<L, 128, true>(tmA, tmB, tmD, tmAux, p, stream);                 \
+    if (BN == 256) return launch_gemm<L, 256, false>(tmA, tmB, tmD, tmAux, p, stream);                   \
+    if (BN == 192) return launch_gemm<L, 192, false>(tmA, tmB, tmD, tmAux, p, stream);                   \
+    return launch_gemm<L, 128, false>(tmA, tmB, tmD, tmAux, p, stream);
   switch (layout) {
     FSB_GEMM_DISPATCH(FSB_GEMM_NT)
     FSB_GEMM_DISPATCH(FSB_GEMM_NN)
diff --git a/fengshen-lm_b200/csrc/ptx.cuh b/fengshen-lm_b200/csrc/ptx.cuh
--- a/fengshen-lm_b200/csrc/ptx.cuh
+++ b/fengshen-lm_b200/csrc/ptx.cuh
@@ -63,7 +63,7 @@
   return reinterpret_cast<uint8_t*>((reinterpret_cast<uintptr_t>(smem_raw) + 1023) & ~uintptr_t(1023));
 }
 
-template <int STAGES, int NFULL = 1>
+template <int STAGES, int NFULL = 1, int RELEASERS = 8>
 struct TmaRing {
   uint64_t* const bar;
   uint64_t* const empty_bar;
@@ -77,7 +77,7 @@
   __device__ __forceinline__ void init() const {
     for (int s = 0; s < STAGES; ++s) {
       for (int f = 0; f < NFULL; ++f) mbar_init(bar + f * STAGES + s, 1);
-      mbar_init(empty(s), 8);
+      mbar_init(empty(s), RELEASERS);
     }
   }
   __device__ __forceinline__ void acquire() const { mbar_wait(empty(stage), phase ^ 1); }
@@ -151,6 +151,7 @@
 template <int N> __device__ __forceinline__ void reg_inc() { asm volatile("setmaxnreg.inc.sync.aligned.u32 %0;" ::"n"(N)); }
 template <int N> __device__ __forceinline__ void reg_dec() { asm volatile("setmaxnreg.dec.sync.aligned.u32 %0;" ::"n"(N)); }
 __device__ __forceinline__ void bar_sync(int id, int n) { asm volatile("bar.sync %0, %1;" ::"r"(id), "r"(n) : "memory"); }
+__device__ __forceinline__ void bar_arrive(int id, int n) { asm volatile("bar.arrive %0, %1;" ::"r"(id), "r"(n) : "memory"); }
 __device__ __forceinline__ float ex2_approx(float x) {
   float y;
   asm("ex2.approx.ftz.f32 %0, %1;" : "=f"(y) : "f"(x));
@@ -217,6 +218,14 @@
       : "+f"(d[0]), "+f"(d[1]), "+f"(d[2]), "+f"(d[3]), "+f"(d[4]), "+f"(d[5]), "+f"(d[6]), "+f"(d[7]), "+f"(d[8]), "+f"(d[9]), "+f"(d[10]), "+f"(d[11]), "+f"(d[12]), "+f"(d[13]), "+f"(d[14]), "+f"(d[15]), "+f"(d[16]), "+f"(d[17]), "+f"(d[18]), "+f"(d[19]), "+f"(d[20]), "+f"(d[21]), "+f"(d[22]), "+f"(d[23]), "+f"(d[24]), "+f"(d[25]), "+f"(d[26]), "+f"(d[27]), "+f"(d[28]), "+f"(d[29]), "+f"(d[30]), "+f"(d[31]), "+f"(d[32]), "+f"(d[33]), "+f"(d[34]), "+f"(d[35]), "+f"(d[36]), "+f"(d[37]), "+f"(d[38]), "+f"(d[39]), "+f"(d[40]), "+f"(d[41]), "+f"(d[42]), "+f"(d[43]), "+f"(d[44]), "+f"(d[45]), "+f"(d[46]), "+f"(d[47]), "+f"(d[48]), "+f"(d[49]), "+f"(d[50]), "+f"(d[51]), "+f"(d[52]), "+f"(d[53]), "+f"(d[54]), "+f"(d[55]), "+f"(d[56]), "+f"(d[57]), "+f"(d[58]), "+f"(d[59]), "+f"(d[60]), "+f"(d[61]), "+f"(d[62]), "+f"(d[63])
       : "l"(da), "l"(db), "r"(accumulate), "n"(kTA), "n"(kTB));
 }
+template <int kTA, int kTB>
+__device__ __forceinline__ void wgmma_ss_n192(float (&d)[96], uint64_t da, uint64_t db, uint32_t accumulate) {
+  asm volatile(
+      "{\n.reg .pred p;\nsetp.ne.b32 p, %98, 0;\n"
+      "wgmma.mma_async.sync.aligned.m64n192k16.f32.bf16.bf16 {%0, %1, %2, %3, %4, %5, %6, %7, %8, %9, %10, %11, %12, %13, %14, %15, %16, %17, %18, %19, %20, %21, %22, %23, %24, %25, %26, %27, %28, %29, %30, %31, %32, %33, %34, %35, %36, %37, %38, %39, %40, %41, %42, %43, %44, %45, %46, %47, %48, %49, %50, %51, %52, %53, %54, %55, %56, %57, %58, %59, %60, %61, %62, %63, %64, %65, %66, %67, %68, %69, %70, %71, %72, %73, %74, %75, %76, %77, %78, %79, %80, %81, %82, %83, %84, %85, %86, %87, %88, %89, %90, %91, %92, %93, %94, %95}, %96, %97, p, 1, 1, %99, %100;\n}"
+      : "+f"(d[0]), "+f"(d[1]), "+f"(d[2]), "+f"(d[3]), "+f"(d[4]), "+f"(d[5]), "+f"(d[6]), "+f"(d[7]), "+f"(d[8]), "+f"(d[9]), "+f"(d[10]), "+f"(d[11]), "+f"(d[12]), "+f"(d[13]), "+f"(d[14]), "+f"(d[15]), "+f"(d[16]), "+f"(d[17]), "+f"(d[18]), "+f"(d[19]), "+f"(d[20]), "+f"(d[21]), "+f"(d[22]), "+f"(d[23]), "+f"(d[24]), "+f"(d[25]), "+f"(d[26]), "+f"(d[27]), "+f"(d[28]), "+f"(d[29]), "+f"(d[30]), "+f"(d[31]), "+f"(d[32]), "+f"(d[33]), "+f"(d[34]), "+f"(d[35]), "+f"(d[36]), "+f"(d[37]), "+f"(d[38]), "+f"(d[39]), "+f"(d[40]), "+f"(d[41]), "+f"(d[42]), "+f"(d[43]), "+f"(d[44]), "+f"(d[45]), "+f"(d[46]), "+f"(d[47]), "+f"(d[48]), "+f"(d[49]), "+f"(d[50]), "+f"(d[51]), "+f"(d[52]), "+f"(d[53]), "+f"(d[54]), "+f"(d[55]), "+f"(d[56]), "+f"(d[57]), "+f"(d[58]), "+f"(d[59]), "+f"(d[60]), "+f"(d[61]), "+f"(d[62]), "+f"(d[63]), "+f"(d[64]), "+f"(d[65]), "+f"(d[66]), "+f"(d[67]), "+f"(d[68]), "+f"(d[69]), "+f"(d[70]), "+f"(d[71]), "+f"(d[72]), "+f"(d[73]), "+f"(d[74]), "+f"(d[75]), "+f"(d[76]), "+f"(d[77]), "+f"(d[78]), "+f"(d[79]), "+f"(d[80]), "+f"(d[81]), "+f"(d[82]), "+f"(d[83]), "+f"(d[84]), "+f"(d[85]), "+f"(d[86]), "+f"(d[87]), "+f"(d[88]), "+f"(d[89]), "+f"(d[90]), "+f"(d[91]), "+f"(d[92]), "+f"(d[93]), "+f"(d[94]), "+f"(d[95])
+      : "l"(da), "l"(db), "r"(accumulate), "n"(kTA), "n"(kTB));
+}
 template <int kTB>
 __device__ __forceinline__ void wgmma_rs_n128(float (&d)[64], const uint32_t (&a)[4], uint64_t db, uint32_t accumulate) {
   asm volatile(
@@ -240,6 +249,13 @@
       "wgmma.mma_async.sync.aligned.m64n256k16.f32.bf16.bf16 {%0, %1, %2, %3, %4, %5, %6, %7, %8, %9, %10, %11, %12, %13, %14, %15, %16, %17, %18, %19, %20, %21, %22, %23, %24, %25, %26, %27, %28, %29, %30, %31, %32, %33, %34, %35, %36, %37, %38, %39, %40, %41, %42, %43, %44, %45, %46, %47, %48, %49, %50, %51, %52, %53, %54, %55, %56, %57, %58, %59, %60, %61, %62, %63, %64, %65, %66, %67, %68, %69, %70, %71, %72, %73, %74, %75, %76, %77, %78, %79, %80, %81, %82, %83, %84, %85, %86, %87, %88, %89, %90, %91, %92, %93, %94, %95, %96, %97, %98, %99, %100, %101, %102, %103, %104, %105, %106, %107, %108, %109, %110, %111, %112, %113, %114, %115, %116, %117, %118, %119, %120, %121, %122, %123, %124, %125, %126, %127}, {%128, %129, %130, %131}, %132, p, 1, 1, %134;\n}"
       : "+f"(d[0]), "+f"(d[1]), "+f"(d[2]), "+f"(d[3]), "+f"(d[4]), "+f"(d[5]), "+f"(d[6]), "+f"(d[7]), "+f"(d[8]), "+f"(d[9]), "+f"(d[10]), "+f"(d[11]), "+f"(d[12]), "+f"(d[13]), "+f"(d[14]), "+f"(d[15]), "+f"(d[16]), "+f"(d[17]), "+f"(d[18]), "+f"(d[19]), "+f"(d[20]), "+f"(d[21]), "+f"(d[22]), "+f"(d[23]), "+f"(d[24]), "+f"(d[25]), "+f"(d[26]), "+f"(d[27]), "+f"(d[28]), "+f"(d[29]), "+f"(d[30]), "+f"(d[31]), "+f"(d[32]), "+f"(d[33]), "+f"(d[34]), "+f"(d[35]), "+f"(d[36]), "+f"(d[37]), "+f"(d[38]), "+f"(d[39]), "+f"(d[40]), "+f"(d[41]), "+f"(d[42]), "+f"(d[43]), "+f"(d[44]), "+f"(d[45]), "+f"(d[46]), "+f"(d[47]), "+f"(d[48]), "+f"(d[49]), "+f"(d[50]), "+f"(d[51]), "+f"(d[52]), "+f"(d[53]), "+f"(d[54]), "+f"(d[55]), "+f"(d[56]), "+f"(d[57]), "+f"(d[58]), "+f"(d[59]), "+f"(d[60]), "+f"(d[61]), "+f"(d[62]), "+f"(d[63]), "+f"(d[64]), "+f"(d[65]), "+f"(d[66]), "+f"(d[67]), "+f"(d[68]), "+f"(d[69]), "+f"(d[70]), "+f"(d[71]), "+f"(d[72]), "+f"(d[73]), "+f"(d[74]), "+f"(d[75]), "+f"(d[76]), "+f"(d[77]), "+f"(d[78]), "+f"(d[79]), "+f"(d[80]), "+f"(d[81]), "+f"(d[82]), "+f"(d[83]), "+f"(d[84]), "+f"(d[85]), "+f"(d[86]), "+f"(d[87]), "+f"(d[88]), "+f"(d[89]), "+f"(d[90]), "+f"(d[91]), "+f"(d[92]), "+f"(d[93]), "+f"(d[94]), "+f"(d[95]), "+f"(d[96]), "+f"(d[97]), "+f"(d[98]), "+f"(d[99]), "+f"(d[100]), "+f"(d[101]), "+f"(d[102]), "+f"(d[103]), "+f"(d[104]), "+f"(d[105]), "+f"(d[106]), "+f"(d[107]), "+f"(d[108]), "+f"(d[109]), "+f"(d[110]), "+f"(d[111]), "+f"(d[112]), "+f"(d[113]), "+f"(d[114]), "+f"(d[115]), "+f"(d[116]), "+f"(d[117]), "+f"(d[118]), "+f"(d[119]), "+f"(d[120]), "+f"(d[121]), "+f"(d[122]), "+f"(d[123]), "+f"(d[124]), "+f"(d[125]), "+f"(d[126]), "+f"(d[127])
       : "r"(a[0]), "r"(a[1]), "r"(a[2]), "r"(a[3]), "l"(db), "r"(accumulate), "n"(kTB));
+}
+template <int N, int kTA, int kTB>
+__device__ __forceinline__ void wgmma_ss_dim(float (&d)[N / 2], uint64_t da, uint64_t db, uint32_t accumulate) {
+  static_assert(N == 128 || N == 192 || N == 256, "no shared-memory-A wrapper for this N");
+  if constexpr (N == 128) wgmma_ss_n128<kTA, kTB>(d, da, db, accumulate);
+  else if constexpr (N == 192) wgmma_ss_n192<kTA, kTB>(d, da, db, accumulate);
+  else wgmma_ss_n256<kTA, kTB>(d, da, db, accumulate);
 }
 template <int N, int kTB>
 __device__ __forceinline__ void wgmma_rs_dim(float (&d)[N / 2], const uint32_t (&a)[4], uint64_t db, uint32_t accumulate) {
```

New measurement: 459,900, median of 6. 1.02x the previous value.
